# Shibodd/volume_path_tracer

Measured on AMD Instinct MI355X. Metric: Msamples/s (whole node) + achieved HBM GB/s, wdas_cloud 1920×1080, higher is better.
Workload: dtype f32

## Files before the change

include/vpt_gpu.h:

```cpp
#ifndef VPT_GPU_H
#define VPT_GPU_H

#include <stddef.h>
#include <stdint.h>

#ifdef __cplusplus
extern "C" {
#endif

#define VPT_ABI_VERSION 1

enum {
  VPT_OK = 0,
  VPT_E_INVALID = 1,
  VPT_E_HIP = 2,
  VPT_E_IO = 3,
  VPT_E_PARSE = 4,
  VPT_E_NOMEM = 5,
  VPT_E_STATE = 6
};


typedef struct vpt_camera_params {
  float position[3];
// ... 88 lines not shown
  uint64_t draws;
  uint64_t stencils;
  uint64_t density_evals;
  uint64_t temp_stencils;
  uint64_t scatters;
  uint64_t shadow_rays;
  uint64_t rng_draws;
  uint64_t exchanged;
} vpt_counters;

int vpt_gpu_create(const vpt_configuration* cfg, const vpt_grid_desc* density,
                   const vpt_grid_desc* temperature, const float* blackbody_500x3, int device,
                   vpt_gpu_ctx** out);
int vpt_gpu_create_many(const vpt_configuration* cfg, const vpt_grid_desc* density,
                        const vpt_grid_desc* temperature, const float* blackbody_500x3, const int* devices, int n,
                        vpt_gpu_ctx** out);
typedef struct vpt_host_grids vpt_host_grids;
int vpt_grids_flatten(const vpt_grid_desc* density, const vpt_grid_desc* temperature, vpt_host_grids** out);
int vpt_gpu_create_from(const vpt_configuration* cfg, const vpt_host_grids* grids, const float* blackbody_500x3,
                        const int* devices, int n, vpt_gpu_ctx** out);
void vpt_grids_free(vpt_host_grids* grids);
int vpt_gpu_destroy(vpt_gpu_ctx* ctx);

int vpt_gpu_job_space(const vpt_gpu_ctx* ctx, uint64_t* jobs_per_wave, uint64_t* total_jobs);

int vpt_gpu_render_jobs(vpt_gpu_ctx* ctx, uint64_t jid_begin, uint64_t jid_count,
                        float* film_device, void* hip_stream);

enum { VPT_FILM_ATOMIC = 0, VPT_FILM_ORDERED = 1 };
int vpt_gpu_set_film_order(vpt_gpu_ctx* ctx, int mode, uint64_t max_bytes);
int vpt_gpu_film_order_info(const vpt_gpu_ctx* ctx, int* mode, uint64_t* buffer_bytes, uint64_t* ordered_launches,
                            uint64_t* atomic_launches);

enum { VPT_POOL_SPARSE = 0, VPT_POOL_DENSE = 1, VPT_POOL_AUTO = 2 };
int vpt_gpu_set_pool_layout(vpt_gpu_ctx* ctx, int layout);
int vpt_gpu_set_pool_cap(vpt_gpu_ctx* ctx, uint64_t max_bytes);
int vpt_gpu_pool_info(const vpt_gpu_ctx* ctx, int* layout, int* policy, uint64_t* sparse_bytes, uint64_t* dense_bytes,
                      double* expand_ms);
int vpt_gpu_debug_read_pool(vpt_gpu_ctx* ctx, int grid, uint64_t cell_begin, uint64_t cell_count, float* out);

int vpt_gpu_render_tiles(vpt_gpu_ctx* ctx, uint32_t tile_lo, uint32_t tile_hi, uint64_t wave_begin,
                         uint64_t wave_count, float* film_device, void* hip_stream);

int vpt_gpu_set_film_moments(vpt_gpu_ctx* ctx, float* m2_device);

int vpt_gpu_render_tile_list(vpt_gpu_ctx* ctx, const uint32_t* tiles, uint32_t n, uint64_t wave_begin,
                             uint64_t wave_count, float* film_device, void* hip_stream);

int vpt_gpu_tile_errors(vpt_gpu_ctx* ctx, const float* film_device, const float* m2_device, float abs_floor,
                        float* err_T_host, void* hip_stream);

typedef struct vpt_adaptive_params {
  float target_error, abs_floor;
  uint32_t min_waves, step_waves, max_waves;
} vpt_adaptive_params;

typedef struct vpt_adaptive_result {
  uint32_t rounds, tiles_at_max;
  uint64_t jobs_rendered, jobs_uniform;
  float max_error;
} vpt_adaptive_result;

int vpt_gpu_render_adaptive(vpt_gpu_ctx* ctx, const vpt_adaptive_params* p, float* film_device, float* m2_device,
                            uint32_t* waves_T_host, float* err_T_host, vpt_adaptive_result* out, void* hip_stream);

int vpt_gpu_render_adaptive_fused(vpt_gpu_ctx* ctx, const vpt_adaptive_params* p, float* film_device, float* m2_device,
// ... 136 lines not shown
```

volume_path_tracer_amd/capi.py:

```python
from __future__ import annotations

import ctypes as C
import os
from pathlib import Path

import numpy as np

PKG_DIR = Path(__file__).resolve().parent
LIB_DIR = PKG_DIR / "lib"
LIB_PATH = Path(os.environ["VPT_LIB"]) if os.environ.get("VPT_LIB") else LIB_DIR / "libvpt_amd.so"

VPT_OK = 0
VPT_BLACKBODY_ROWS = 500


class CameraParams(C.Structure):
    _fields_ = [("position", C.c_float * 3), ("look", C.c_float * 3), ("up", C.c_float * 3),
                ("vfov_deg", C.c_float), ("imaging_ratio", C.c_float)]


class WorkerParams(C.Structure):
    _fields_ = [("single_pixel_enabled", C.c_int32), ("use_jitter", C.c_int32),
                ("single_pixel_coord", C.c_int64 * 2),
                ("infinite_light_xyz", C.c_float * 3), ("infinite_light_multiplier", C.c_float),
# ... 66 lines not shown
    def as_dict(self) -> dict:
        return {n: (float if n == "max_error" else int)(getattr(self, n)) for n, _ in self._fields_}


class DenoiseParams(C.Structure):
    _fields_ = [("iterations", C.c_uint32), ("n_guides", C.c_uint32), ("sigma_l", C.c_float), ("rel_floor", C.c_float),
                ("guide_sigma", C.c_float * 4)]

    @classmethod
    def make(cls, iterations=4, n_guides=0, sigma_l=4.0, rel_floor=1e-3, guide_sigma=None):
        if guide_sigma is None:
            guide_sigma = 0.2
        if np.isscalar(guide_sigma):
            guide_sigma = [guide_sigma] * n_guides
        gs = [float(v) for v in guide_sigma][:4]
        if len(gs) < min(n_guides, 4):
            raise ValueError("denoise: one guide_sigma per guide")
        gs += [1.0] * (4 - len(gs))
        return cls(int(iterations), int(n_guides), float(sigma_l), float(rel_floor), (C.c_float * 4)(*gs))


assert C.sizeof(DenoiseParams) == 32

EVENT_DTYPE = np.dtype([("jid", "<u8"), ("pixel", "<u4"), ("seq", "<u4"), ("type", "<u4"), ("v", "<f4", (7,))])
assert EVENT_DTYPE.itemsize == 48
DDA_ROW_DTYPE = np.dtype([("ijk", "<i4", (3,)), ("t", "<f4"), ("value", "<f4"), ("dim_getdim", "<u4"),
                          ("dim_nodeinfo", "<u4"), ("active", "<i4"), ("maximum", "<f4")])
assert DDA_ROW_DTYPE.itemsize == 36
VPT_RNG_REFERENCE, VPT_RNG_PIXEL = 0, 1
VPT_ORDER_JID, VPT_ORDER_COST_WAVE_MAJOR, VPT_ORDER_COST_TILE_MAJOR, VPT_ORDER_COST_TAIL = 0, 1, 2, 3
VPT_ORDER_COST_SAME_TILE = 4
VPT_FILM_ATOMIC, VPT_FILM_ORDERED = 0, 1
VPT_POOL_SPARSE, VPT_POOL_DENSE, VPT_POOL_AUTO = 0, 1, 2
VPT_GATES_CONTEXT, VPT_GATES_LATENCY, VPT_GATES_FULL = 0, 1, 2
EVENT_NAMES = ("new_ray", "sampled_point", "null", "scatter_terminated", "scatter", "absorbed")


def _ptr(arr, ctype):
    if arr is None:
        return C.cast(None, C.POINTER(ctype))
    return arr.ctypes.data_as(C.POINTER(ctype))


class Grid:

    def __init__(self, *, map_mat, map_inv_mat, map_vec, background, bbox_min, bbox_max,
                 leaf_origin, leaf_values, leaf_max, leaf_value_mask=None,
                 tile_origin=None, tile_level=None, tile_value=None, tile_active=None,
                 lower_origin=None, upper_origin=None):
        self.leaf_origin = np.ascontiguousarray(leaf_origin, dtype=np.int32).reshape(-1, 3)
        n = self.leaf_origin.shape[0]
        self.leaf_values = np.ascontiguousarray(leaf_values, dtype=np.float32).reshape(n, 512)
        self.leaf_max = np.ascontiguousarray(leaf_max, dtype=np.float32).reshape(n)
        if leaf_value_mask is None:
            leaf_value_mask = np.full((n, 8), np.uint64(0xFFFFFFFFFFFFFFFF), dtype=np.uint64)
        self.leaf_value_mask = np.ascontiguousarray(leaf_value_mask, dtype=np.uint64).reshape(n, 8)
        self.tile_origin = None if tile_origin is None else np.ascontiguousarray(tile_origin, dtype=np.int32).reshape(-1, 3)
        self.tile_level = None if tile_level is None else np.ascontiguousarray(tile_level, dtype=np.int32)
        self.tile_value = None if tile_value is None else np.ascontiguousarray(tile_value, dtype=np.float32)
        self.tile_active = None if tile_active is None else np.ascontiguousarray(tile_active, dtype=np.uint8)
        self.lower_origin = None if lower_origin is None else np.ascontiguousarray(lower_origin, dtype=np.int32).reshape(-1, 3)
        self.upper_origin = None if upper_origin is None else np.ascontiguousarray(upper_origin, dtype=np.int32).reshape(-1, 3)
        d = GridDesc()
        d.map_mat[:] = [float(x) for x in np.asarray(map_mat, dtype=np.float32).reshape(9)]
        d.map_inv_mat[:] = [float(x) for x in np.asarray(map_inv_mat, dtype=np.float32).reshape(9)]
        d.map_vec[:] = [float(x) for x in np.asarray(map_vec, dtype=np.float32).reshape(3)]
# ... 108 lines not shown
        L.vpt_gpu_denoise.argtypes = [vp, C.POINTER(DenoiseParams), vp, vp, C.POINTER(vp), vp, vp, vp]
    L.vpt_gpu_sync.argtypes = [vp]
    L.vpt_gpu_film_clear.argtypes = [vp]
    L.vpt_gpu_film_device_ptr.argtypes = [vp, C.POINTER(vp), C.POINTER(C.c_uint64)]
    L.vpt_gpu_film_add_to_host.argtypes = [vp, fp]
    L.vpt_gpu_counters.argtypes = [vp, C.POINTER(Counters), C.c_int]
    L.vpt_gpu_profile.argtypes = [vp, C.POINTER(C.c_uint64), C.c_int, C.c_int]
    L.vpt_gpu_set_tuning.argtypes = [vp, C.c_int, C.c_int, C.c_int, C.c_int, C.c_int]
    if hasattr(L, "vpt_gpu_set_latency_tuning"):
        L.vpt_gpu_set_latency_tuning.argtypes = [vp, C.c_int, C.c_int, C.c_int, C.c_int, C.c_int]
    if hasattr(L, "vpt_gpu_set_full_tuning"):
        L.vpt_gpu_set_full_tuning.argtypes = [vp, C.c_int, C.c_int, C.c_int, C.c_int]
    if hasattr(L, "vpt_gpu_gate_info"):
        L.vpt_gpu_gate_info.argtypes = [vp, C.c_int, C.POINTER(C.c_int), C.POINTER(C.c_int)]
    L.vpt_gpu_launch_info.argtypes = [vp, C.POINTER(C.c_int), C.POINTER(C.c_int)]
    L.vpt_last_error.restype = C.c_char_p
    L.vpt_synth_grid.argtypes = [C.c_int, C.c_int]
    L.vpt_synth_grid.restype = gridp
    L.vpt_synth_free.argtypes = [gridp]
    L.vpt_grid_from_nanovdb.argtypes = [C.c_void_p, C.c_size_t, C.POINTER(gridp)]
    L.vpt_grid_read_nvdb.argtypes = [C.c_char_p, C.c_char_p, C.POINTER(gridp)]
    L.vpt_grid_free.argtypes = [gridp]
    L.vpt_film_to_srgb8.argtypes = [fp, C.c_int64, C.c_int64, C.POINTER(C.c_uint8)]
    L.vpt_gpu_trace_jobs.argtypes = [vp, C.c_uint64, C.c_uint64, vp, vp, C.c_uint64, C.POINTER(C.c_uint64), vp]
    L.vpt_gpu_majorant_trace.argtypes = [vp, fp, fp, fp, C.c_int, C.POINTER(C.c_int)]
    L.vpt_dda_trace.argtypes = [C.POINTER(GridDesc), fp, fp, vp, C.c_int, C.POINTER(C.c_int)]
    L.vpt_gpu_set_rng_mode.argtypes = [vp, C.c_int]
    if hasattr(L, "vpt_gpu_set_pixel_chunk"):
        L.vpt_gpu_set_pixel_chunk.argtypes = [vp, C.c_int]
    L.vpt_gpu_set_run_skipping.argtypes = [vp, C.c_int]
    L.vpt_gpu_kernel_variant.argtypes = [vp, C.POINTER(C.c_int), C.POINTER(C.c_int)]
    if hasattr(L, "vpt_gpu_last_launch_variant"):
        L.vpt_gpu_last_launch_variant.argtypes = [vp, C.POINTER(C.c_int)]
    if hasattr(L, "vpt_gpu_set_film_order"):
        L.vpt_gpu_set_film_order.argtypes = [vp, C.c_int, C.c_uint64]
        L.vpt_gpu_film_order_info.argtypes = [vp, C.POINTER(C.c_int), C.POINTER(C.c_uint64),
                                              C.POINTER(C.c_uint64), C.POINTER(C.c_uint64)]
    if hasattr(L, "vpt_gpu_set_pool_layout"):
        L.vpt_gpu_set_pool_layout.argtypes = [vp, C.c_int]
        L.vpt_gpu_set_pool_cap.argtypes = [vp, C.c_uint64]
        L.vpt_gpu_pool_info.argtypes = [vp, C.POINTER(C.c_int), C.POINTER(C.c_int), C.POINTER(C.c_uint64),
                                        C.POINTER(C.c_uint64), C.POINTER(C.c_double)]
        L.vpt_gpu_debug_read_pool.argtypes = [vp, C.c_int, C.c_uint64, C.c_uint64, fp]
    L.vpt_gpu_set_job_order.argtypes = [vp, C.c_int]
    L.vpt_gpu_set_job_order_tail.argtypes = [vp, C.c_int]
    L.vpt_gpu_tile_costs.argtypes = [vp, fp, C.POINTER(C.c_uint32)]
    L.vpt_gpu_set_tile_costs.argtypes = [vp, fp]
    L.vpt_gpu_set_job_permutation.argtypes = [vp, C.POINTER(C.c_uint32), C.c_uint64]
    if hasattr(L, "vpt_gpu_set_latency_kernel"):
        L.vpt_gpu_set_latency_kernel.argtypes = [vp, C.c_int, C.c_int]
    if hasattr(L, "vpt_gpu_set_compaction"):
        L.vpt_gpu_set_compaction.argtypes = [vp, C.c_int]
        L.vpt_gpu_latency_kernel_info.argtypes = [vp, C.POINTER(C.c_int), C.POINTER(C.c_int)]
    if hasattr(L, "vpt_gpu_bind_thread_near"):
        L.vpt_gpu_bind_thread_near.argtypes = [vp, C.POINTER(C.c_int)]
    if hasattr(L, "vpt_gpu_stream_create"):
        L.vpt_gpu_stream_create.argtypes = [vp, C.POINTER(vp)]
        L.vpt_gpu_stream_destroy.argtypes = [vp, vp]
        L.vpt_gpu_stream_sync.argtypes = [vp, vp]
        L.vpt_gpu_film_alloc.argtypes = [vp, C.POINTER(vp)]
        L.vpt_gpu_film_free.argtypes = [vp, vp]
        L.vpt_gpu_film_flush_to_host.argtypes = [vp, vp, fp]
    if hasattr(L, "vpt_gpu_feed_open"):
        L.vpt_gpu_feed_open.argtypes = [vp, vp, vp, C.c_uint64, C.POINTER(vp)]
        L.vpt_gpu_feed_push.argtypes = [vp, C.POINTER(C.c_uint64), C.c_uint64]
        L.vpt_gpu_feed_close.argtypes = [vp]
# ... 45 lines not shown
```

volume_path_tracer_amd/csrc/vpt_ctx.h:

```cpp
#pragma once

#include <hip/hip_runtime.h>

#include <atomic>
#include <chrono>
#include <cstdint>
#include <mutex>
#include <string>
#include <vector>

#include "vpt_internal.h"
#include "vpt_launch.h"

#define VPT_HIP(call)                                                                                 \
  do {                                                                                                \
    hipError_t e_ = (call);                                                                           \
    if (e_ != hipSuccess)                                                                             \
      return ::vpt::set_error(VPT_E_HIP, std::string(#call " failed: ") + hipGetErrorString(e_));            \
  } while (0)

#ifndef VPT_DEFAULT_JOB_ORDER
#define VPT_DEFAULT_JOB_ORDER VPT_ORDER_COST_SAME_TILE
#endif

#ifndef VPT_DEFAULT_FULL_GATE_IDLE
#define VPT_DEFAULT_FULL_GATE_IDLE 4
#endif

#ifndef VPT_RUNS_MIN_FRACTION
#define VPT_RUNS_MIN_FRACTION 0.25
#endif

namespace vpt {
struct DeviceGrid {
  void* cells8 = nullptr;
  void* runs8 = nullptr;
  void* walk8 = nullptr;
  double run_fraction = 0.0;
  void* cells128 = nullptr;
  void* root = nullptr;
  void* bricks = nullptr;
  void* dense = nullptr;
  DevGrid dev{};
  size_t bytes = 0;
  size_t brick_bytes = 0, dense_bytes = 0;
};

}

namespace vpt {
struct FeedLaunch {
  const uint64_t* word;
  uint64_t* ring;
  uint64_t mask;
  unsigned* error;
  uint64_t* started;
  uint64_t* waiting;
  uint32_t* tile_done;
};
struct BandLaunch {
  uint32_t tile_lo, tiles, waves, group;
  bool list = false;
};
}

struct vpt_gpu_feed;

struct vpt_gpu_ctx {
  int device = 0;
  vpt_configuration cfg{};
  vpt::DevScene scene{};
  vpt::DeviceGrid density, temperature;
  float* bb = nullptr;
  float* cie = nullptr;
  float* film = nullptr;
  uint64_t film_count = 0;
  unsigned long long* job_counter = nullptr;
  hipEvent_t slot_done[64] = {};
  bool slot_used[64] = {};
  uint32_t next_slot = 0;
  std::mutex slot_mu;
  unsigned long long* counters = nullptr;
  unsigned long long* prof = nullptr;
  vpt::DevScene* scene_dev = nullptr;
  vpt::DevScene* scene_lat_dev = nullptr;
  int lat_gate[4] = {1, 65, 1, 1};
  int lat_wave_lanes = 0;
  vpt::DevScene* scene_full_dev = nullptr;
  int full_gate[4] = {0, 0, 0, 0};
  int last_gate_set = -1;
  int last_eval_split = -1;
  hipStream_t stream = nullptr;
  bool use_runs = false;
  int pixel_chunk = 0;
  int grid_blocks = 0;
  int cus = 1;
  bool grid_user = false;
  int order_mode = VPT_DEFAULT_JOB_ORDER;
  int order_tail_waves = 0;
  uint32_t* order = nullptr;
  std::vector<float> tile_cost;
  uint32_t* perm = nullptr;
  uint64_t perm_n = 0;
  std::vector<uint32_t> tile_rank;
  float* staging = nullptr;
  std::vector<vpt_gpu_feed*> feed_pool;
  std::atomic<int> open_feeds{0};
  float* zeros = nullptr;
  int lat_mode = -1;
  int lat_ungated = 0;
  int lat_per_cu = 1;
  int compact_every = 0;
  int compact_per_cu = 0;
  int film_order = VPT_FILM_ORDERED;
  uint64_t film_order_max = 0;
  float* samples = nullptr;
  uint64_t samples_bytes = 0;
  hipEvent_t samples_done = nullptr;
  bool samples_used = false;
  uint64_t ordered_launches = 0, atomic_launches = 0;
  uint32_t* band_rank = nullptr;
  uint32_t band_rank_lo = 0, band_rank_hi = 0;
  uint32_t* list_dev = nullptr;
  uint32_t* list_slot_dev = nullptr;
  std::vector<uint32_t> list_host, list_slot_host;
  bool list_ranked = false;
  float* m2 = nullptr;
  float* tile_err = nullptr;
  float* gang_scratch = nullptr;
  uint64_t gang_scratch_bytes = 0;
  uint32_t* gang_waves = nullptr;
  void* denoise_scratch = nullptr;
  uint64_t denoise_scratch_bytes = 0;
  hipEvent_t denoise_done = nullptr;
  bool denoise_used = false;
  std::mutex denoise_mu;
  uint64_t frame_waves = 0, frame_jid_lo = 0;
  uint32_t frame_tile_lo = 0, frame_tiles = 0;
  float* frame_film = nullptr;
  double setup_ms[5] = {};
  int pool_policy = VPT_POOL_AUTO;
  uint64_t pool_cap = 0;
  float pool_expand_ms = 0.0f;
};

struct vpt_gpu_feed {
  vpt_gpu_ctx* ctx = nullptr;
  hipStream_t stream = nullptr;
  float* film = nullptr;
  uint64_t* block = nullptr;
  uint64_t* word = nullptr;
  uint32_t* error = nullptr;
  uint64_t* started = nullptr;
// ... 35 lines not shown
```

volume_path_tracer_amd/csrc/vpt_gpu.hip:

```cpp
#include <hip/hip_runtime.h>
#include <pthread.h>
#include <sched.h>
#include <unistd.h>

#include <algorithm>
#include <cmath>
#include <cstdio>
#include <cstdlib>
#include <cstring>
#include <fstream>
#include <functional>
#include <memory>
#include <atomic>
#include <mutex>
#include <chrono>
#include <string>
#include <thread>
#include <vector>

#include "vpt_ctx.h"
#include "vpt_kernels.h"
#include "vpt_denoise.h"

namespace vpt {
// ... 293 lines not shown
    VPT_HIP(hipEventCreate(&ev[0]));
    VPT_HIP(hipEventCreate(&ev[1]));
    (void)hipEventRecord(ev[0], nullptr);
    for (vpt::DeviceGrid* d : grids)
      if (d && rc == VPT_OK) rc = vpt::expand_dense(*d);
    (void)hipEventRecord(ev[1], nullptr);
    const hipError_t e = hipEventSynchronize(ev[1]);
    if (rc == VPT_OK && e != hipSuccess) rc = vpt::set_error(VPT_E_HIP, std::string("dense stencil pool: ") + hipGetErrorString(e));
    if (rc == VPT_OK) (void)hipEventElapsedTime(&ctx->pool_expand_ms, ev[0], ev[1]);
    (void)hipEventDestroy(ev[0]);
    (void)hipEventDestroy(ev[1]);
    if (rc != VPT_OK) {
      dense = false;
      if (rc == VPT_E_NOMEM && policy == VPT_POOL_AUTO) rc = VPT_OK;
    }
  }
  for (vpt::DeviceGrid* d : grids) {
    if (!d) continue;
    if (!dense) vpt::free_dense(*d);
    d->dev.dense = (const float*)d->dense;
  }
  ctx->scene.density.dense = ctx->density.dev.dense;
  ctx->scene.temperature.dense = ctx->temperature.dev.dense;
  return rc;
}

int default_pool_policy() {
  const char* v = std::getenv("VPT_POOL_LAYOUT");
  if (v && !std::strcmp(v, "sparse")) return VPT_POOL_SPARSE;
  if (v && !std::strcmp(v, "dense")) return VPT_POOL_DENSE;
  return VPT_POOL_AUTO;
}

}

int vpt::host::ctx_device(vpt_gpu_ctx* ctx) {
  hipError_t e = hipSetDevice(ctx->device);
  if (e != hipSuccess) return vpt::set_error(VPT_E_HIP, std::string("hipSetDevice: ") + hipGetErrorString(e));
  return VPT_OK;
}

int vpt::host::launch_tile_counts(vpt_gpu_ctx* ctx, float* film, const uint32_t* counts_dev, hipStream_t s) {
  const uint64_t npix = (uint64_t)ctx->scene.W * (uint64_t)ctx->scene.H;
  hipLaunchKernelGGL(vpt::vpt_tile_count_kernel, dim3((unsigned)((npix + 255) / 256)), dim3(256), 0, s, ctx->scene_dev,
                     film, counts_dev);
  VPT_HIP(hipGetLastError());
  return VPT_OK;
}

int vpt::host::render(vpt_gpu_ctx* ctx, uint64_t jid_begin, uint64_t jid_count, float* film, float* records,
                      void* stream_ptr, vpt_event* events, uint64_t event_cap, uint32_t* slot_out,
                      const vpt::FeedLaunch* feed, const vpt::BandLaunch* band) {
  if (!ctx) return vpt::set_error(VPT_E_INVALID, "render: null context");
  int rc = ctx_device(ctx);
  if (rc) return rc;
  if (jid_count == 0) return VPT_OK;
  if (feed && (ctx->scene.pixel_mode || records || events))
    return vpt::set_error(VPT_E_INVALID, "render: feeds run the reference RNG mode's production kernels only");
  if (band && (feed || records || events || ctx->scene.pixel_mode || ctx->film_order != VPT_FILM_ORDERED || ctx->frame_waves))
    return vpt::set_error(VPT_E_INVALID, "render: band launches are ordered production launches of the reference RNG mode");
  const uint64_t per_job = (uint64_t)ctx->scene.tile_area * 3 * sizeof(float);
  const bool ordered = ctx->film_order == VPT_FILM_ORDERED && !feed && !records && !events && !ctx->scene.pixel_mode;
  if (ctx->m2 && !feed && (!ordered || ctx->frame_waves))
    return vpt::set_error(VPT_E_STATE, "render: a moment plane is attached and this launch would add with film atomics (" +
                                           std::string(ctx->frame_waves ? "a frame is open"
                                                       : records || events ? "a debug launch"
                                                                           : "not an ordered launch of the reference RNG mode") +
                                           "): detach it (vpt_gpu_set_film_moments NULL)");
  if (ordered && !band) {
    const uint64_t max_jobs = std::min<uint64_t>(ordered_cap(ctx, jid_count * per_job) / per_job, 0xffffffffULL);
    if (max_jobs == 0) return vpt::set_error(VPT_E_NOMEM, "ordered film: no room for one job's samples");
    if (jid_count > max_jobs) {
      const uint64_t T = ctx->scene.T;
      const uint64_t chunk = max_jobs >= T ? max_jobs / T * T : max_jobs;
      for (uint64_t b = 0; b < jid_count; b += chunk)
        if ((rc = render(ctx, jid_begin + b, std::min(chunk, jid_count - b), film, nullptr, stream_ptr))) return rc;
      return VPT_OK;
    }
  }
  const uint64_t total = ctx->scene.T * (uint64_t)ctx->cfg.num_waves;
  (void)total;
  hipStream_t s = (hipStream_t)stream_ptr;
  vpt::KernelArgs env{};
  env.jid_begin = jid_begin;
  env.jid_count = jid_count;
  env.pixel_chunk = 1;
  if (ctx->scene.pixel_mode) {
    const uint64_t area = ctx->scene.tile_area;
    if (jid_count > UINT64_MAX / area) return vpt::set_error(VPT_E_INVALID, "render: job range too large");
    const uint64_t items = jid_count * area;
    uint64_t K = 1;
    if (ctx->pixel_chunk > 0) {
      K = (uint64_t)ctx->pixel_chunk;
    } else {
      const uint64_t lanes = (uint64_t)ctx->grid_blocks * vpt::kBlockThreads;
      while (area % (2 * K) == 0 && items / (2 * K) >= 32 * lanes) K *= 2;
    }
    env.pixel_chunk = (uint32_t)K;
    env.jid_count = items / K;
  }
  env.film = film ? film : ctx->film;
  env.records = records;
  env.tile_area = ctx->scene.tw * ctx->scene.th;
  env.prof_buf = ctx->prof;
  env.order = nullptr;
  env.perm = nullptr;
  env.order_tail_k0 = 0;
  env.order_tail_n = 0;
  env.order_group = vpt::kOrderGroup;
  uint32_t blocks = (uint32_t)ctx->grid_blocks;
  const bool latency = env.jid_count <= kSpreadLanes * ((uint64_t)blocks * (vpt::kBlockThreads / 64));
  const uint64_t cus = (uint64_t)ctx->cus;
  if (!ctx->grid_user && !latency) {
    const uint64_t resident_per_cu = std::max<uint64_t>(1, blocks / cus);
    const double x = (double)env.jid_count / ((double)blocks * vpt::kBlockThreads);
    const uint64_t per_cu = std::min<uint64_t>(resident_per_cu, (uint64_t)std::max(1.0, std::floor(1.5 + 1.8 * x)));
    blocks = (uint32_t)std::min<uint64_t>(blocks, cus * per_cu);
  }
#ifdef VPT_JOB_LOG
  const bool temp = ctx->scene.has_temperature != 0, dbg = events != nullptr;
#else
  const bool temp = ctx->scene.has_temperature != 0, dbg = records != nullptr || events != nullptr;
#endif
  const uint64_t lat_blocks = cus * (uint64_t)ctx->lat_per_cu;
  const bool use_lat = !dbg && !feed && ctx->lat_mode != 0 &&
                       (ctx->lat_mode == 1 || (!ctx->grid_user && (latency || blocks <= lat_blocks)));
  if (use_lat) blocks = (uint32_t)std::min<uint64_t>(latency ? lat_blocks : blocks, lat_blocks);
  const bool compact = use_lat && !latency && ctx->compact_every > 0 &&
                       (uint64_t)blocks <= cus * (uint64_t)std::max(0, ctx->compact_per_cu);
  const uint64_t T = ctx->scene.T;
  if (band) {
    if ((rc = ensure_order(ctx))) return rc;
  } else if (!feed && ctx->order_mode != VPT_ORDER_JID && jid_begin % T == 0 && jid_count % T == 0 && jid_count < (1ULL << 32)) {
    if ((rc = ensure_order(ctx))) return rc;
    const uint32_t n = (uint32_t)(jid_count / T);
    uint32_t tail = 0;
    const bool same_tile = ctx->order_mode == VPT_ORDER_COST_SAME_TILE && ordered && !ctx->frame_waves &&
                           !(use_lat && !latency);
    if (ctx->order_mode == VPT_ORDER_COST_TILE_MAJOR || same_tile) tail = n;
    if (same_tile) env.order_group = 1;
    if (ctx->order_mode == VPT_ORDER_COST_TAIL || (ctx->order_mode == VPT_ORDER_COST_SAME_TILE && !same_tile)) {
      const uint64_t lanes = (uint64_t)blocks * vpt::kBlockThreads;
      const uint64_t want = ctx->order_tail_waves > 0 ? (uint64_t)ctx->order_tail_waves : (6 * lanes + T - 1) / T;
      tail = (uint32_t)std::min<uint64_t>(n, want);
    }
    env.order = ctx->order;
    env.order_tail_n = tail;
    env.order_tail_k0 = (n - tail) * (uint32_t)T;
  }
  if (!feed && !band && ctx->perm && ctx->perm_n == jid_count && !ctx->scene.pixel_mode) env.perm = ctx->perm;
  float* samples = nullptr;
  if (band) {
    const uint64_t bytes = vpt::band_sample_floats(band->tiles, band->waves, ctx->scene.tile_area, band->group) * sizeof(float);
    if ((rc = ensure_samples(ctx, bytes, samples))) return rc;
    if (!samples)
      return vpt::set_error(VPT_E_STATE, "vpt_gpu_render_tiles: the sample buffer would have to grow (" +
                                             std::to_string(bytes >> 20) + " MiB) while a feed of the context is open");
  } else if (ordered && !ctx->frame_waves && (rc = ensure_samples(ctx, jid_count * per_job, samples))) {
    return rc;
  }
  if (ctx->m2 && !feed && !samples)
    return vpt::set_error(VPT_E_STATE, "render: a moment plane is attached and the sample buffer would have to grow while "
                                       "a feed of the context is open (the launch would add with film atomics)");
  env.samples = samples;
  if (samples) {
    ++ctx->ordered_launches;
    if (ctx->samples_used) VPT_HIP(hipStreamWaitEvent(s, ctx->samples_done, 0));
  } else if (!feed) {
    ++ctx->atomic_launches;
  }
  if (band) {
    env.band_rank = ctx->order;
    env.band_slot_map = nullptr;
    if (band->list) {
      if (!ctx->band_rank || !ctx->list_dev || !ctx->list_slot_dev)
        return vpt::set_error(VPT_E_NOMEM, "vpt_gpu_render_tile_list: no tile-list buffers (their allocation failed)");
      if (!ctx->list_ranked) {
        hipLaunchKernelGGL(vpt::vpt_band_rank_kernel, dim3(1), dim3(256), 0, s, ctx->order, (uint32_t)T, 0u, band->tiles,
                           ctx->band_rank, ctx->list_slot_dev);
        VPT_HIP(hipGetLastError());
        ctx->band_rank_lo = ctx->band_rank_hi = 0;
        ctx->list_ranked = true;
      }
      env.band_rank = ctx->band_rank;
      env.band_slot_map = ctx->list_slot_dev;
    } else if (band->tile_lo != 0 || band->tiles != T) {
      if (!ctx->band_rank) return vpt::set_error(VPT_E_NOMEM, "vpt_gpu_render_tiles: no tile-rank buffer (its allocation failed)");
      if (ctx->band_rank_lo != band->tile_lo || ctx->band_rank_hi != band->tile_lo + band->tiles) {
        hipLaunchKernelGGL(vpt::vpt_band_rank_kernel, dim3(1), dim3(256), 0, s, ctx->order, (uint32_t)T, band->tile_lo,
                           band->tile_lo + band->tiles, ctx->band_rank, (const uint32_t*)nullptr);
        VPT_HIP(hipGetLastError());
        ctx->band_rank_lo = band->tile_lo;
        ctx->band_rank_hi = band->tile_lo + band->tiles;
// ... 50 lines not shown
                                         : vpt::vpt_integrate_kernel<false, false, false, false, false, false, true>;
      if (scene == ctx->scene_dev) scene = ctx->scene_full_dev;
      hipLaunchKernelGGL(kernel, dim3(blocks), dim3(vpt::kBlockThreads), 0, s, env, scene, ctx->counters);
    }
  } else if (use_lat) {
    env.compact_every = (uint32_t)std::max(1, ctx->compact_every);
    if (compact) {
      auto kernel = temp ? vpt::vpt_integrate_kernel<true, false, false, true, true>
                         : ctx->use_runs ? vpt::vpt_integrate_kernel<false, false, true, true, true>
                                         : vpt::vpt_integrate_kernel<false, false, false, true, true>;
      hipLaunchKernelGGL(kernel, dim3(blocks), dim3(vpt::kBlockThreads), vpt::kXchgBytes, s, env, scene, ctx->counters);
    } else {
      auto kernel = temp ? vpt::vpt_integrate_kernel<true, false, false, true>
                         : ctx->use_runs ? vpt::vpt_integrate_kernel<false, false, true, true>
                                         : vpt::vpt_integrate_kernel<false, false, false, true>;
      hipLaunchKernelGGL(kernel, dim3(blocks), dim3(vpt::kBlockThreads), 0, s, env, scene, ctx->counters);
    }
  } else if (feed) {
    auto kernel = temp ? vpt::vpt_integrate_kernel<true, false, false, false, false, true>
                       : ctx->use_runs ? vpt::vpt_integrate_kernel<false, false, true, false, false, true>
                                       : vpt::vpt_integrate_kernel<false, false, false, false, false, true>;
    hipLaunchKernelGGL(kernel, dim3(blocks), dim3(vpt::kBlockThreads), 0, s, env, scene, ctx->counters);
  } else {
    auto kernel = temp ? (dbg ? vpt::vpt_integrate_kernel<true, true, false> : vpt::vpt_integrate_kernel<true, false, false>)
                       : ctx->use_runs
                           ? (dbg ? vpt::vpt_integrate_kernel<false, true, true> : vpt::vpt_integrate_kernel<false, false, true>)
                           : (dbg ? vpt::vpt_integrate_kernel<false, true, false> : vpt::vpt_integrate_kernel<false, false, false>);
    if (!dbg && scene == ctx->scene_dev) scene = ctx->scene_full_dev;
    hipLaunchKernelGGL(kernel, dim3(blocks), dim3(vpt::kBlockThreads), 0, s, env, scene, ctx->counters);
  }
  ctx->last_gate_set = scene == ctx->scene_full_dev ? VPT_GATES_FULL
                       : scene == ctx->scene_lat_dev ? VPT_GATES_LATENCY : VPT_GATES_CONTEXT;
  ctx->last_eval_split = vpt::kernel_eval_split(temp, dbg, use_lat) ? 1 : 0;
  VPT_HIP(hipGetLastError());
  const uint64_t npix = (uint64_t)ctx->scene.W * (uint64_t)ctx->scene.H;
  if (band) {
    const uint32_t chunks = (ctx->scene.tile_area + 63u) / 64u;
    const uint32_t* const list = band->list ? ctx->list_dev : nullptr;
    hipLaunchKernelGGL(ctx->m2 ? vpt::vpt_band_order_kernel<true> : vpt::vpt_band_order_kernel<false>,
                       dim3(band->tiles * chunks), dim3(64), 0, s, ctx->scene_dev, env.film, (const float*)samples,
                       band->tile_lo, band->waves, env.band_groups, band->group, list, ctx->m2);
    VPT_HIP(hipGetLastError());
    VPT_HIP(hipEventRecord(ctx->samples_done, s));
    ctx->samples_used = true;
  } else if (samples) {
    const uint64_t threads = ctx->scene.T * (uint64_t)ctx->scene.tile_area;
    hipLaunchKernelGGL(ctx->m2 ? vpt::vpt_film_order_kernel<true> : vpt::vpt_film_order_kernel<false>,
                       dim3((unsigned)((threads + 255) / 256)), dim3(256), 0, s, ctx->scene_dev, env.film,
                       (const float*)samples, jid_begin, jid_count, ctx->m2);
    VPT_HIP(hipGetLastError());
    VPT_HIP(hipEventRecord(ctx->samples_done, s));
    ctx->samples_used = true;
  } else if (!feed) {
    hipLaunchKernelGGL(vpt::vpt_count_kernel, dim3((unsigned)((npix + 255) / 256)), dim3(256), 0, s, ctx->scene_dev,
                       env.film, jid_begin, jid_count);
    VPT_HIP(hipGetLastError());
  }
  return release_slot(ctx, s, slot);
}

extern "C" {

const char* vpt_last_error(void) { return vpt::g_last_error.c_str(); }
int vpt_abi_version(void) { return VPT_ABI_VERSION; }

int vpt_gpu_device_count(int* count) {
// ... 68 lines not shown
  if (trc) return vpt::set_error(trc, tmsg);
  g.has_temperature = temperature != nullptr;
  if (ms) *ms += std::chrono::duration<double, std::milli>(std::chrono::steady_clock::now() - t0).count();
  return VPT_OK;
}

int create_on(const vpt_configuration* cfg, const HostGrids& grids, const float* blackbody_500x3, int device,
              vpt_gpu_ctx** out) {
  *out = nullptr;
  std::unique_ptr<vpt_gpu_ctx, void (*)(vpt_gpu_ctx*)> ctx(new vpt_gpu_ctx(), destroy);
  ctx->device = device;
  ctx->cfg = *cfg;
  ctx->setup_ms[0] = grids.flatten_ms;
  using clk = std::chrono::steady_clock;
  auto t = clk::now();
  auto lap = [&](int i) {
    const auto now = clk::now();
    ctx->setup_ms[i] += std::chrono::duration<double, std::milli>(now - t).count();
    t = now;
  };
  int rc = ctx_device(ctx.get());
  if (rc) return rc;
  lap(4);
  if ((rc = vpt::build_scene(*cfg, ctx->scene))) return rc;
  if ((rc = vpt::upload_grid(grids.density, ctx->density))) return rc;
  if (grids.has_temperature && (rc = vpt::upload_grid(grids.temperature, ctx->temperature))) return rc;
  lap(1);
  const bool has_temperature = grids.has_temperature;
  ctx->use_runs = !has_temperature && ctx->density.run_fraction >= VPT_RUNS_MIN_FRACTION;
  ctx->scene.density = ctx->density.dev;
  vpt::scene_finalize(ctx->scene);
  ctx->scene.temperature = ctx->temperature.dev;
  ctx->scene.has_temperature = has_temperature ? 1 : 0;
  ctx->pool_policy = default_pool_policy();
  if ((rc = apply_pool_layout(ctx.get(), ctx->pool_policy))) return rc;
  lap(1);
  ctx->scene.bb_lds_ok = has_temperature ? vpt::blackbody_rows_suffice(grids.temp_range, cfg->volume_parameters.temperature_scale,
                                                                    cfg->volume_parameters.temperature_offset, vpt::kBbLdsRows)
                                     : 0;

  std::vector<float> bb(501 * 3, 0.0f);
  if (blackbody_500x3)
    std::memcpy(bb.data(), blackbody_500x3, 500 * 3 * sizeof(float));
  else
    vpt::blackbody_table(bb.data());
  size_t scratch = 0;
  if ((rc = vpt::upload(bb.data(), bb.size() * sizeof(float), (void**)&ctx->bb, scratch))) return rc;
  if ((rc = vpt::upload(vpt::cie_table(), 471 * 3 * sizeof(float), (void**)&ctx->cie, scratch))) return rc;
  ctx->scene.bb = ctx->bb;
  ctx->scene.cie = ctx->cie;

  ctx->film_count = (uint64_t)cfg->output_size[0] * (uint64_t)cfg->output_size[1] * 4;
  VPT_HIP(hipMalloc((void**)&ctx->film, ctx->film_count * sizeof(float)));
  VPT_HIP(hipMemset(ctx->film, 0, ctx->film_count * sizeof(float)));
  VPT_HIP(hipMalloc((void**)&ctx->job_counter, kLaunchSlots * 2 * sizeof(unsigned long long)));
  for (uint32_t i = 0; i < kLaunchSlots; ++i)
    VPT_HIP(hipEventCreateWithFlags(&ctx->slot_done[i], hipEventDisableTiming));
  VPT_HIP(hipMalloc((void**)&ctx->counters, vpt::kCounterCount * sizeof(unsigned long long)));
  VPT_HIP(hipMemset(ctx->counters, 0, vpt::kCounterCount * sizeof(unsigned long long)));
  VPT_HIP(hipMalloc((void**)&ctx->prof, kProfWords * sizeof(unsigned long long)));
  VPT_HIP(hipMemset(ctx->prof, 0, kProfWords * sizeof(unsigned long long)));
  VPT_HIP(hipStreamCreateWithFlags(&ctx->stream, hipStreamNonBlocking));
  VPT_HIP(hipEventCreateWithFlags(&ctx->samples_done, hipEventDisableTiming));

  int per_cu = 0, cus = 0;
  VPT_HIP(hipOccupancyMaxActiveBlocksPerMultiprocessor(
// ... 584 lines not shown
  ctx->scene.pixel_mode = mode == VPT_RNG_PIXEL ? 1 : 0;
  ctx->scene.tile_area = (uint32_t)(ctx->scene.tw * ctx->scene.th);
  return push_scene(ctx);
}

int vpt_gpu_set_pixel_chunk(vpt_gpu_ctx* ctx, int chunk) {
  if (!ctx || chunk < 0 || (chunk & (chunk - 1)) != 0 || (chunk > 0 && ctx->scene.tile_area % (uint32_t)chunk != 0))
    return vpt::set_error(VPT_E_INVALID, "vpt_gpu_set_pixel_chunk: 0 or a power of two dividing the tile area");
  ctx->pixel_chunk = chunk;
  return VPT_OK;
}

int vpt_gpu_set_run_skipping(vpt_gpu_ctx* ctx, int mode) {
  if (!ctx || mode < -1 || mode > 1) return vpt::set_error(VPT_E_INVALID, "vpt_gpu_set_run_skipping: bad argument");
  if (mode == 1 && ctx->scene.has_temperature)
    return vpt::set_error(VPT_E_INVALID, "vpt_gpu_set_run_skipping: no run-skipping variant with a temperature grid");
  ctx->use_runs = mode < 0 ? (!ctx->scene.has_temperature && ctx->density.run_fraction >= VPT_RUNS_MIN_FRACTION) : mode == 1;
  return VPT_OK;
}

int vpt_gpu_kernel_variant(const vpt_gpu_ctx* ctx, int* has_temperature, int* run_skipping) {
  if (!ctx) return vpt::set_error(VPT_E_INVALID, "null context");
  if (has_temperature) *has_temperature = ctx->scene.has_temperature ? 1 : 0;
  if (run_skipping) *run_skipping = ctx->use_runs ? 1 : 0;
  return VPT_OK;
}

int vpt_gpu_last_launch_variant(const vpt_gpu_ctx* ctx, int* eval_split) {
  if (!ctx) return vpt::set_error(VPT_E_INVALID, "null context");
  if (eval_split) *eval_split = ctx->last_eval_split;
  return VPT_OK;
}

int vpt_gpu_set_pool_layout(vpt_gpu_ctx* ctx, int layout) {
  if (!ctx || layout < VPT_POOL_SPARSE || layout > VPT_POOL_AUTO)
    return vpt::set_error(VPT_E_INVALID, "vpt_gpu_set_pool_layout: bad argument");
  if (ctx->open_feeds.load() > 0) return vpt::set_error(VPT_E_STATE, "vpt_gpu_set_pool_layout: a feed of this context is open");
  if (ctx->frame_waves) return vpt::set_error(VPT_E_STATE, "vpt_gpu_set_pool_layout: a frame is open");
  int rc = ctx_device(ctx);
  if (rc) return rc;
  if ((rc = wait_ctx(ctx))) return rc;
  VPT_HIP(hipDeviceSynchronize());
  ctx->pool_policy = layout;
  rc = apply_pool_layout(ctx, layout);
  const int prc = push_scene(ctx);
  return rc ? rc : prc;
}

int vpt_gpu_set_pool_cap(vpt_gpu_ctx* ctx, uint64_t max_bytes) {
  if (!ctx) return vpt::set_error(VPT_E_INVALID, "vpt_gpu_set_pool_cap: null context");
  ctx->pool_cap = max_bytes;
  return VPT_OK;
}

int vpt_gpu_pool_info(const vpt_gpu_ctx* ctx, int* layout, int* policy, uint64_t* sparse_bytes, uint64_t* dense_bytes,
                      double* expand_ms) {
  if (!ctx) return vpt::set_error(VPT_E_INVALID, "null context");
  if (layout) *layout = ctx->density.dense ? VPT_POOL_DENSE : VPT_POOL_SPARSE;
  if (policy) *policy = ctx->pool_policy;
  if (sparse_bytes) sparse_bytes[0] = ctx->density.brick_bytes, sparse_bytes[1] = ctx->temperature.brick_bytes;
  if (dense_bytes) dense_bytes[0] = ctx->density.dense_bytes, dense_bytes[1] = ctx->temperature.dense_bytes;
  if (expand_ms) *expand_ms = ctx->pool_expand_ms;
  return VPT_OK;
}

int vpt_gpu_debug_read_pool(vpt_gpu_ctx* ctx, int grid, uint64_t cell_begin, uint64_t cell_count, float* out) {
// ... 438 lines not shown
```

volume_path_tracer_amd/csrc/vpt_integrator.h:

```cpp
#pragma once

#include <hip/hip_runtime.h>
#include <stdint.h>

#include "vpt_math.h"

namespace vpt {

struct RootTileDev {
  int32_t origin[3];
  float value;
  int32_t active;
  int32_t pad[3];
};

struct DevGrid {
  float mat[9], inv_mat[9], vec[3];
  float background;
  int32_t bbox_min[3], bbox_max[3];
  int32_t r8_org[3], r8_n[3];
  int32_t w8_org[3], w8_n[3];
  uint32_t w8_max;
  int32_t r128_org[3], r128_n[3];
  int32_t root_count, leaf_count;
// ... 957 lines not shown
    return (uint64_t)w * T + order[k - w * T];
  }
  k -= tail_k0;
  const uint32_t full = T / group, span = group * tail_n;
  uint32_t w, i;
  if (k < full * span) {
    const uint32_t g = k / span, r = k - g * span;
    w = r / group;
    i = g * group + (r - w * group);
  } else {
    const uint32_t R = T - full * group, r = k - full * span;
    w = r / R;
    i = full * group + (r - w * R);
  }
  return (uint64_t)(tail_k0 / T + w) * T + order[i];
}

constexpr uint32_t kBandGroup = 64;
__host__ __device__ __forceinline__ uint64_t band_job(uint64_t k, uint32_t waves, uint32_t T, const uint32_t* band_rank) {
  const uint64_t i = k / waves;
  const uint32_t w = (uint32_t)(k - i * waves);
  return (uint64_t)w * T + band_rank[i];
}
__host__ __device__ __forceinline__ uint32_t band_groups(uint32_t waves, uint32_t G) { return (waves + G - 1) / G; }
__host__ __device__ __forceinline__ uint64_t band_slot(uint32_t tb, uint32_t w, uint32_t q, uint32_t groups,
                                                       uint32_t tile_area, uint32_t G) {
  const uint32_t g = w / G;
  return (((((uint64_t)tb * groups + g) * tile_area + q) * G) + (w - g * G)) * 3;
}
__host__ __device__ __forceinline__ uint64_t band_sample_floats(uint32_t tiles, uint32_t waves, uint32_t tile_area,
                                                                uint32_t G) {
  return (uint64_t)tiles * band_groups(waves, G) * tile_area * G * 3;
}

__host__ __device__ __forceinline__ void lane_park(Lane& ln) {
  ln.sm = SM_NONE;
  ln.shadow = 0;
  for (int i = 0; i < 3; ++i) {
    ln.e[i] = ln.d[i] = ln.nxt[i] = ln.finc[i] = 0.0f;
    ln.vox[i] = ln.vinc[i] = 0;
  }
  ln.scale = ln.rscale = ln.maj = ln.Tn = ln.T1 = ln.s_t0 = ln.s_t1 = ln.s_dmaj = 0.0f;
  ln.dim = 0;
  ln.pw = 0;
}

template <class Env, class = void>
struct env_is_gang {
  static constexpr bool value = false;
};
template <class Env>
struct env_is_gang<Env, decltype((void)Env::kGang)> {
  static constexpr bool value = Env::kGang;
};


template <bool Debug, class Env>
__host__ __device__ __forceinline__ void nee_done(const DevScene& S, Lane& ln, LaneCold& lc, Env& env) {
  env.prof(PB_NEE_DONE);
  if (lc.Tr >= 0.0f) {
    float c = lc.rd[0] * S.wi[0] + (lc.rd[1] * S.wi[1] + lc.rd[2] * S.wi[2]);
    float p = hg_eval(S, c);
    float pt = p * lc.Tr;
    lc.L[0] = lc.L[0] + pt * S.Li[0];
    lc.L[1] = lc.L[1] + pt * S.Li[1];
    lc.L[2] = lc.L[2] + pt * S.Li[2];
// ... 385 lines not shown
```

volume_path_tracer_amd/render.py:

```python
from __future__ import annotations

import ctypes as C
import threading
import time
from typing import Optional

import numpy as np

from . import capi


def ceildiv(a: int, b: int) -> int:
    return a // b + (a % b != 0)


class TileProvider:

    def __init__(self, img_size, waves: int, tile_size):
        self.img_w, self.img_h = int(img_size[0]), int(img_size[1])
        self.tile_w, self.tile_h = int(tile_size[0]), int(tile_size[1])
        self.ntx, self.nty = ceildiv(self.img_w, self.tile_w), ceildiv(self.img_h, self.tile_h)
        self.num_tiles = self.ntx * self.nty
        self.requested_waves = int(waves)
        self.max_wave_idx = 0
# ... 257 lines not shown
                   "vpt_gpu_majorant_trace")
        if n.value > max_rows:
            raise RuntimeError(f"majorant_trace: {n.value} segments exceed max_rows {max_rows}")
        return rows[: n.value].copy()

    def set_rng_mode(self, mode: int) -> None:
        capi.check(capi.lib().vpt_gpu_set_rng_mode(self.h, int(mode)), "vpt_gpu_set_rng_mode")

    def set_pixel_chunk(self, chunk: int) -> None:
        capi.check(capi.lib().vpt_gpu_set_pixel_chunk(self.h, int(chunk)), "vpt_gpu_set_pixel_chunk")

    def set_run_skipping(self, mode: int) -> None:
        capi.check(capi.lib().vpt_gpu_set_run_skipping(self.h, int(mode)), "vpt_gpu_set_run_skipping")

    def set_latency_kernel(self, mode: int, ungated: int = -1) -> None:
        capi.check(capi.lib().vpt_gpu_set_latency_kernel(self.h, int(mode), int(ungated)), "vpt_gpu_set_latency_kernel")

    def set_compaction(self, every: int) -> None:
        capi.check(capi.lib().vpt_gpu_set_compaction(self.h, int(every)), "vpt_gpu_set_compaction")

    def latency_kernel_info(self) -> dict:
        m, b = C.c_int(), C.c_int()
        capi.check(capi.lib().vpt_gpu_latency_kernel_info(self.h, C.byref(m), C.byref(b)), "vpt_gpu_latency_kernel_info")
        return {"mode": int(m.value), "resident_blocks_per_cu": int(b.value)}

    def kernel_variant(self, last_launch: bool = False) -> dict:
        t, r = C.c_int(), C.c_int()
        capi.check(capi.lib().vpt_gpu_kernel_variant(self.h, C.byref(t), C.byref(r)), "vpt_gpu_kernel_variant")
        kv = {"has_temperature": bool(t.value), "run_skipping": bool(r.value)}
        if last_launch:
            e = C.c_int()
            capi.check(capi.lib().vpt_gpu_last_launch_variant(self.h, C.byref(e)), "vpt_gpu_last_launch_variant")
            kv["eval_split"] = None if e.value < 0 else bool(e.value)
        return kv

    def set_film_order(self, mode: int, max_bytes: int = 0) -> None:
        capi.check(capi.lib().vpt_gpu_set_film_order(self.h, int(mode), int(max_bytes)), "vpt_gpu_set_film_order")

    def film_order_info(self) -> dict:
        m, b, o, a = C.c_int(), C.c_uint64(), C.c_uint64(), C.c_uint64()
        capi.check(capi.lib().vpt_gpu_film_order_info(self.h, C.byref(m), C.byref(b), C.byref(o), C.byref(a)),
                   "vpt_gpu_film_order_info")
        return {"mode": int(m.value), "buffer_bytes": int(b.value), "ordered_launches": int(o.value),
                "atomic_launches": int(a.value)}

    def set_pool_layout(self, layout: int, cap_bytes: int | None = None) -> None:
        if cap_bytes is not None:
            capi.check(capi.lib().vpt_gpu_set_pool_cap(self.h, int(cap_bytes)), "vpt_gpu_set_pool_cap")
        capi.check(capi.lib().vpt_gpu_set_pool_layout(self.h, int(layout)), "vpt_gpu_set_pool_layout")

    def pool_info(self) -> dict:
        la, po, ms = C.c_int(), C.c_int(), C.c_double()
        sp, de = (C.c_uint64 * 2)(), (C.c_uint64 * 2)()
        capi.check(capi.lib().vpt_gpu_pool_info(self.h, C.byref(la), C.byref(po), sp, de, C.byref(ms)), "vpt_gpu_pool_info")
        return {"layout": int(la.value), "policy": int(po.value), "sparse_bytes": (int(sp[0]), int(sp[1])),
                "dense_bytes": (int(de[0]), int(de[1])), "expand_ms": float(ms.value)}

    def debug_read_pool(self, grid: int, cell_begin: int, cell_count: int) -> np.ndarray:
        out = np.empty((int(cell_count), 2304), dtype=np.float32)
        capi.check(capi.lib().vpt_gpu_debug_read_pool(self.h, int(grid), int(cell_begin), int(cell_count),
                                                      out.ctypes.data_as(C.POINTER(C.c_float))), "vpt_gpu_debug_read_pool")
        return out

    def set_job_order(self, mode: int) -> None:
        capi.check(capi.lib().vpt_gpu_set_job_order(self.h, int(mode)), "vpt_gpu_set_job_order")

    def set_job_order_tail(self, waves: int) -> None:
# ... 190 lines not shown
```

Measured before the change: 1737.

## Route ordered whole-wave job launches through the lane-major band sample layout

In ordered-film mode with same-tile job ordering, whole-wave job-range launches are now re-expressed as band launches. They use the lane-grouped sample layout that tile renders already use, and are chunked by wave groups to fit the ordered-buffer cap. This aims to give more coalesced sample writes and a cheaper reduction into the film than the per-job sample layout. The routing falls back to the job layout if the buffer cannot grow, latency kernels are in use, or a permutation or feed is active. An environment variable and an API call can force the old layout.

```diff
diff --git a/include/vpt_gpu.h b/include/vpt_gpu.h
--- a/include/vpt_gpu.h
+++ b/include/vpt_gpu.h
@@ -144,6 +144,11 @@
 int vpt_gpu_film_order_info(const vpt_gpu_ctx* ctx, int* mode, uint64_t* buffer_bytes, uint64_t* ordered_launches,
                             uint64_t* atomic_launches);
 
+enum { VPT_SAMPLES_AUTO = 0, VPT_SAMPLES_JOB = 1 };
+int vpt_gpu_set_sample_layout(vpt_gpu_ctx* ctx, int mode);
+enum { VPT_LAYOUT_JOB = 0, VPT_LAYOUT_LANE = 1 };
+int vpt_gpu_last_launch_layout(const vpt_gpu_ctx* ctx, int* layout, int* mode);
+
 enum { VPT_POOL_SPARSE = 0, VPT_POOL_DENSE = 1, VPT_POOL_AUTO = 2 };
 int vpt_gpu_set_pool_layout(vpt_gpu_ctx* ctx, int layout);
 int vpt_gpu_set_pool_cap(vpt_gpu_ctx* ctx, uint64_t max_bytes);
diff --git a/volume_path_tracer_amd/capi.py b/volume_path_tracer_amd/capi.py
--- a/volume_path_tracer_amd/capi.py
+++ b/volume_path_tracer_amd/capi.py
@@ -122,6 +122,8 @@
 VPT_ORDER_COST_SAME_TILE = 4
 VPT_FILM_ATOMIC, VPT_FILM_ORDERED = 0, 1
 VPT_POOL_SPARSE, VPT_POOL_DENSE, VPT_POOL_AUTO = 0, 1, 2
+VPT_SAMPLES_AUTO, VPT_SAMPLES_JOB = 0, 1
+VPT_LAYOUT_JOB, VPT_LAYOUT_LANE = 0, 1
 VPT_GATES_CONTEXT, VPT_GATES_LATENCY, VPT_GATES_FULL = 0, 1, 2
 EVENT_NAMES = ("new_ray", "sampled_point", "null", "scatter_terminated", "scatter", "absorbed")
 
@@ -296,6 +298,9 @@
     L.vpt_gpu_kernel_variant.argtypes = [vp, C.POINTER(C.c_int), C.POINTER(C.c_int)]
     if hasattr(L, "vpt_gpu_last_launch_variant"):
         L.vpt_gpu_last_launch_variant.argtypes = [vp, C.POINTER(C.c_int)]
+    if hasattr(L, "vpt_gpu_set_sample_layout"):
+        L.vpt_gpu_set_sample_layout.argtypes = [vp, C.c_int]
+        L.vpt_gpu_last_launch_layout.argtypes = [vp, C.POINTER(C.c_int), C.POINTER(C.c_int)]
     if hasattr(L, "vpt_gpu_set_film_order"):
         L.vpt_gpu_set_film_order.argtypes = [vp, C.c_int, C.c_uint64]
         L.vpt_gpu_film_order_info.argtypes = [vp, C.POINTER(C.c_int), C.POINTER(C.c_uint64),
diff --git a/volume_path_tracer_amd/csrc/vpt_ctx.h b/volume_path_tracer_amd/csrc/vpt_ctx.h
--- a/volume_path_tracer_amd/csrc/vpt_ctx.h
+++ b/volume_path_tracer_amd/csrc/vpt_ctx.h
@@ -21,6 +21,10 @@
 
 #ifndef VPT_DEFAULT_JOB_ORDER
 #define VPT_DEFAULT_JOB_ORDER VPT_ORDER_COST_SAME_TILE
+#endif
+
+#ifndef VPT_DEFAULT_SAMPLE_LAYOUT
+#define VPT_DEFAULT_SAMPLE_LAYOUT VPT_SAMPLES_AUTO
 #endif
 
 #ifndef VPT_DEFAULT_FULL_GATE_IDLE
@@ -61,6 +65,7 @@
 struct BandLaunch {
   uint32_t tile_lo, tiles, waves, group;
   bool list = false;
+  bool routed = false;
 };
 }
 
@@ -119,6 +124,8 @@
   hipEvent_t samples_done = nullptr;
   bool samples_used = false;
   uint64_t ordered_launches = 0, atomic_launches = 0;
+  int sample_layout = VPT_DEFAULT_SAMPLE_LAYOUT;
+  int last_sample_layout = -1;
   uint32_t* band_rank = nullptr;
   uint32_t band_rank_lo = 0, band_rank_hi = 0;
   uint32_t* list_dev = nullptr;
diff --git a/volume_path_tracer_amd/csrc/vpt_gpu.hip b/volume_path_tracer_amd/csrc/vpt_gpu.hip
--- a/volume_path_tracer_amd/csrc/vpt_gpu.hip
+++ b/volume_path_tracer_amd/csrc/vpt_gpu.hip
@@ -349,6 +349,13 @@
   return VPT_POOL_AUTO;
 }
 
+int default_sample_layout() {
+  const char* v = std::getenv("VPT_SAMPLE_LAYOUT");
+  if (v && !std::strcmp(v, "job")) return VPT_SAMPLES_JOB;
+  if (v && !std::strcmp(v, "auto")) return VPT_SAMPLES_AUTO;
+  return VPT_DEFAULT_SAMPLE_LAYOUT;
+}
+
 }
 
 int vpt::host::ctx_device(vpt_gpu_ctx* ctx) {
@@ -384,11 +391,31 @@
                                                        : records || events ? "a debug launch"
                                                                            : "not an ordered launch of the reference RNG mode") +
                                            "): detach it (vpt_gpu_set_film_moments NULL)");
-  if (ordered && !band) {
+  const uint64_t T = ctx->scene.T;
+  const vpt::BandLaunch* const routed = band && band->routed ? band : nullptr;
+  if (routed) band = nullptr;
+  vpt::BandLaunch offer{};
+  if (ordered && !band && !routed && ctx->sample_layout == VPT_SAMPLES_AUTO && ctx->order_mode == VPT_ORDER_COST_SAME_TILE &&
+      !ctx->frame_waves && ctx->open_feeds.load() == 0 && vpt::lane_range_ok(jid_begin, jid_count, T, vpt::kBandGroup) &&
+      !(ctx->perm && ctx->perm_n == jid_count)) {
+    const uint64_t G = vpt::kBandGroup, waves = jid_count / T, per_wave = T * per_job;
+    const uint64_t max_waves = ordered_cap(ctx, (waves + G - 1) / G * G * per_wave) / per_wave;
+    if (max_waves > 0) {
+      const uint64_t chunk = vpt::lane_chunk(max_waves, (uint32_t)G);
+      for (uint64_t b = 0; b < waves && waves > chunk; b += chunk) {
+        const uint64_t n = std::min(chunk, waves - b);
+        const vpt::BandLaunch part{0u, (uint32_t)T, (uint32_t)n, vpt::lane_group(max_waves, n, (uint32_t)G), false, true};
+        if ((rc = render(ctx, jid_begin + b * T, n * T, film, nullptr, stream_ptr, nullptr, 0, nullptr, nullptr, &part))) return rc;
+      }
+      if (waves > chunk) return VPT_OK;
+      offer = vpt::BandLaunch{0u, (uint32_t)T, (uint32_t)waves, vpt::lane_group(max_waves, waves, (uint32_t)G), false, true};
+    }
+  }
+  const vpt::BandLaunch* const lane_offer = routed ? routed : offer.routed ? &offer : nullptr;
+  if (ordered && !band && !routed) {
     const uint64_t max_jobs = std::min<uint64_t>(ordered_cap(ctx, jid_count * per_job) / per_job, 0xffffffffULL);
     if (max_jobs == 0) return vpt::set_error(VPT_E_NOMEM, "ordered film: no room for one job's samples");
     if (jid_count > max_jobs) {
-      const uint64_t T = ctx->scene.T;
       const uint64_t chunk = max_jobs >= T ? max_jobs / T * T : max_jobs;
       for (uint64_t b = 0; b < jid_count; b += chunk)
         if ((rc = render(ctx, jid_begin + b, std::min(chunk, jid_count - b), film, nullptr, stream_ptr))) return rc;
@@ -445,15 +472,32 @@
   if (use_lat) blocks = (uint32_t)std::min<uint64_t>(latency ? lat_blocks : blocks, lat_blocks);
   const bool compact = use_lat && !latency && ctx->compact_every > 0 &&
                        (uint64_t)blocks <= cus * (uint64_t)std::max(0, ctx->compact_per_cu);
-  const uint64_t T = ctx->scene.T;
+  const bool whole_waves = !feed && ctx->order_mode != VPT_ORDER_JID && jid_begin % T == 0 && jid_count % T == 0 &&
+                           jid_count < (1ULL << 32);
+  float* samples = nullptr;
+  if (band) {
+    const uint64_t bytes = vpt::band_sample_floats(band->tiles, band->waves, ctx->scene.tile_area, band->group) * sizeof(float);
+    if ((rc = ensure_samples(ctx, bytes, samples))) return rc;
+    if (!samples)
+      return vpt::set_error(VPT_E_STATE, "vpt_gpu_render_tiles: the sample buffer would have to grow (" +
+                                             std::to_string(bytes >> 20) + " MiB) while a feed of the context is open");
+  } else if (ordered && !ctx->frame_waves) {
+    if (lane_offer && whole_waves && !use_lat) {
+      const uint64_t bytes =
+          vpt::band_sample_floats(lane_offer->tiles, lane_offer->waves, ctx->scene.tile_area, lane_offer->group) * sizeof(float);
+      if (ensure_samples(ctx, bytes, samples) != VPT_OK) samples = nullptr;
+      if (samples) band = lane_offer;
+    }
+    if (!band && (rc = ensure_samples(ctx, jid_count * per_job, samples))) return rc;
+  }
   if (band) {
     if ((rc = ensure_order(ctx))) return rc;
-  } else if (!feed && ctx->order_mode != VPT_ORDER_JID && jid_begin % T == 0 && jid_count % T == 0 && jid_count < (1ULL << 32)) {
+  } else if (whole_waves) {
     if ((rc = ensure_order(ctx))) return rc;
     const uint32_t n = (uint32_t)(jid_count / T);
     uint32_t tail = 0;
     const bool same_tile = ctx->order_mode == VPT_ORDER_COST_SAME_TILE && ordered && !ctx->frame_waves &&
-                           !(use_lat && !latency);
+                           samples != nullptr && !(use_lat && !latency);
     if (ctx->order_mode == VPT_ORDER_COST_TILE_MAJOR || same_tile) tail = n;
     if (same_tile) env.order_group = 1;
     if (ctx->order_mode == VPT_ORDER_COST_TAIL || (ctx->order_mode == VPT_ORDER_COST_SAME_TILE && !same_tile)) {
@@ -466,16 +510,6 @@
     env.order_tail_k0 = (n - tail) * (uint32_t)T;
   }
   if (!feed && !band && ctx->perm && ctx->perm_n == jid_count && !ctx->scene.pixel_mode) env.perm = ctx->perm;
-  float* samples = nullptr;
-  if (band) {
-    const uint64_t bytes = vpt::band_sample_floats(band->tiles, band->waves, ctx->scene.tile_area, band->group) * sizeof(float);
-    if ((rc = ensure_samples(ctx, bytes, samples))) return rc;
-    if (!samples)
-      return vpt::set_error(VPT_E_STATE, "vpt_gpu_render_tiles: the sample buffer would have to grow (" +
-                                             std::to_string(bytes >> 20) + " MiB) while a feed of the context is open");
-  } else if (ordered && !ctx->frame_waves && (rc = ensure_samples(ctx, jid_count * per_job, samples))) {
-    return rc;
-  }
   if (ctx->m2 && !feed && !samples)
     return vpt::set_error(VPT_E_STATE, "render: a moment plane is attached and the sample buffer would have to grow while "
                                        "a feed of the context is open (the launch would add with film atomics)");
@@ -592,6 +626,7 @@
   ctx->last_gate_set = scene == ctx->scene_full_dev ? VPT_GATES_FULL
                        : scene == ctx->scene_lat_dev ? VPT_GATES_LATENCY : VPT_GATES_CONTEXT;
   ctx->last_eval_split = vpt::kernel_eval_split(temp, dbg, use_lat) ? 1 : 0;
+  ctx->last_sample_layout = band ? VPT_LAYOUT_LANE : VPT_LAYOUT_JOB;
   VPT_HIP(hipGetLastError());
   const uint64_t npix = (uint64_t)ctx->scene.W * (uint64_t)ctx->scene.H;
   if (band) {
@@ -726,6 +761,7 @@
   vpt::scene_finalize(ctx->scene);
   ctx->scene.temperature = ctx->temperature.dev;
   ctx->scene.has_temperature = has_temperature ? 1 : 0;
+  ctx->sample_layout = default_sample_layout();
   ctx->pool_policy = default_pool_policy();
   if ((rc = apply_pool_layout(ctx.get(), ctx->pool_policy))) return rc;
   lap(1);
@@ -1376,6 +1412,20 @@
   return VPT_OK;
 }
 
+int vpt_gpu_set_sample_layout(vpt_gpu_ctx* ctx, int mode) {
+  if (!ctx || (mode != VPT_SAMPLES_AUTO && mode != VPT_SAMPLES_JOB))
+    return vpt::set_error(VPT_E_INVALID, "vpt_gpu_set_sample_layout: bad argument");
+  ctx->sample_layout = mode;
+  return VPT_OK;
+}
+
+int vpt_gpu_last_launch_layout(const vpt_gpu_ctx* ctx, int* layout, int* mode) {
+  if (!ctx) return vpt::set_error(VPT_E_INVALID, "null context");
+  if (layout) *layout = ctx->last_sample_layout;
+  if (mode) *mode = ctx->sample_layout;
+  return VPT_OK;
+}
+
 int vpt_gpu_set_pool_layout(vpt_gpu_ctx* ctx, int layout) {
   if (!ctx || layout < VPT_POOL_SPARSE || layout > VPT_POOL_AUTO)
     return vpt::set_error(VPT_E_INVALID, "vpt_gpu_set_pool_layout: bad argument");
diff --git a/volume_path_tracer_amd/csrc/vpt_integrator.h b/volume_path_tracer_amd/csrc/vpt_integrator.h
--- a/volume_path_tracer_amd/csrc/vpt_integrator.h
+++ b/volume_path_tracer_amd/csrc/vpt_integrator.h
@@ -1013,6 +1013,17 @@
                                                                 uint32_t G) {
   return (uint64_t)tiles * band_groups(waves, G) * tile_area * G * 3;
 }
+__host__ __device__ __forceinline__ bool lane_range_ok(uint64_t jid_begin, uint64_t jid_count, uint64_t T, uint32_t G) {
+  if (T == 0 || jid_count == 0 || jid_begin % T != 0 || jid_count % T != 0) return false;
+  const uint64_t waves = jid_count / T;
+  return waves < (1ULL << 32) && (waves + G - 1) / G * G * T < (1ULL << 32);
+}
+__host__ __device__ __forceinline__ uint64_t lane_chunk(uint64_t max_waves, uint32_t G) {
+  return max_waves >= G ? max_waves / G * G : max_waves;
+}
+__host__ __device__ __forceinline__ uint32_t lane_group(uint64_t max_waves, uint64_t part_waves, uint32_t G) {
+  return max_waves >= G ? G : (uint32_t)part_waves;
+}
 
 __host__ __device__ __forceinline__ void lane_park(Lane& ln) {
   ln.sm = SM_NONE;
diff --git a/volume_path_tracer_amd/render.py b/volume_path_tracer_amd/render.py
--- a/volume_path_tracer_amd/render.py
+++ b/volume_path_tracer_amd/render.py
@@ -313,7 +313,14 @@
             e = C.c_int()
             capi.check(capi.lib().vpt_gpu_last_launch_variant(self.h, C.byref(e)), "vpt_gpu_last_launch_variant")
             kv["eval_split"] = None if e.value < 0 else bool(e.value)
+            la = C.c_int(-1)
+            if hasattr(capi.lib(), "vpt_gpu_last_launch_layout"):
+                capi.check(capi.lib().vpt_gpu_last_launch_layout(self.h, C.byref(la), None), "vpt_gpu_last_launch_layout")
+            kv["sample_layout"] = {capi.VPT_LAYOUT_JOB: "job", capi.VPT_LAYOUT_LANE: "lane"}.get(la.value)
         return kv
+
+    def set_sample_layout(self, mode: int) -> None:
+        capi.check(capi.lib().vpt_gpu_set_sample_layout(self.h, int(mode)), "vpt_gpu_set_sample_layout")
 
     def set_film_order(self, mode: int, max_bytes: int = 0) -> None:
         capi.check(capi.lib().vpt_gpu_set_film_order(self.h, int(mode), int(max_bytes)), "vpt_gpu_set_film_order")
```

After: 1749 (median of 6 runs). About the same (+0.7%).
